# kscalelabs/gym-kmanip

Measured on AMD Instinct MI355X. Metric: env steps/sec (whole node), KManipSoloArm @4096 envs, 1/2/4/8 MI355X, higher is better.
Workload: dtype f64

## Files before the change

### gym_kmanip_amd/csrc/kmanip_api.hip

```cpp
#include <hip/hip_runtime.h>

#include <cstdio>
#include <cstdlib>
#include <cmath>
#include <cstring>
#include <new>
#include <string>
#include <vector>

#include "kmanip_device.hpp"

#define KM_VERSION "kmanip-hip 0.37 (gfx950, f64)"

static thread_local std::string g_create_error;

struct KHandle_ {
  KModelDesc desc;
  KDeviceModel* dmodel = nullptr;
  KDeviceState st{};
  int device = 0;
  int num_envs = 0;
  std::string err;
  std::vector<hipEvent_t> ev;
  std::vector<char> ev_render;
  bool timing = false;
  int timing_every = 1;
  long timing_count = 0;
  double* rd_rec[2] = {nullptr, nullptr};
  int rd_sel = 0;
  int timed_steps = 0;
  double* qpos_snap[2] = {nullptr, nullptr};
  int render_src = -1;
  bool last_step_timed = false;
  int step_cam = -1, step_h = 0, step_w = 0;
  float* step_depth = nullptr;
  int epb_forced = 0;
  int32_t* slot_env = nullptr;
  bool cost_sort = false;
  KCostWeights cost_w{18, 1, 2000, 0, 0, 100};
  uint8_t* spread_flags[2] = {nullptr, nullptr};
  unsigned spread_k = 0;
  int last_epb = 0;
  double* envp_buf = nullptr;
  double* ep_range_buf = nullptr;
  int* ep_flag = nullptr;
  KVisArgs vis{};
  double* vp_buf = nullptr;
  double* vp_range_buf = nullptr;
  int* vp_flag = nullptr;
  int32_t* ep_snap[2] = {nullptr, nullptr};
  bool ep_snap_ok[2] = {false, false};
  std::vector<KLinkCapsule> links;
  KLinkCapsule* links_buf = nullptr;
  bool depth_links = false;
  unsigned long long* index_errors = nullptr;
  double* stage_buf = nullptr;
  int32_t* stage_cnt = nullptr;
  int stage_cap = 0;
  std::vector<void*> allocs;
};

struct DevGuard {
  int prev = -1;
  bool ok = true;
  explicit DevGuard(int dev) {
// ... 1119 lines not shown
```

### gym_kmanip_amd/csrc/kmanip_dyn_newton.hpp

```cpp
#pragma once

enum { KM_SUB_ALL = 0, KM_SUB_ARM = 1, KM_SUB_CUBE = 2 };
template <int NL, int S> struct SubSet {
  static constexpr int D0 = S == KM_SUB_CUBE ? NL : 0, D1 = S == KM_SUB_ARM ? NL : NL + 6;
  static constexpr int kind(int c) { return slot_kind<NL>(c); }
  static constexpr bool slot(int c) { return S == KM_SUB_ALL || (S == KM_SUB_ARM ? kind(c) == 2 : kind(c) == 0); }
  static constexpr int c0(int c) { const int k = kind(c); const int lo = k == 0 ? NL : 0; return lo > D0 ? lo : D0; }
  static constexpr int c1(int c) { const int k = kind(c); const int hi = k == 2 ? NL : NL + 6; return hi < D1 ? hi : D1; }
};

template <int G, int N, int D0, int D1>
__device__ __forceinline__ void chol_rows(real (&h)[N], real& invd, int sub, int& bad) {
  static_for<D0, D1>([&](auto kc) {
    constexpr int k = decltype(kc)::value;
    real dk = gbcast<G, k>(h[k]);
    if (!(dk > 0)) { bad = 1; dk = 1; }
    const real inv = rsqrt_nr(dk);
    const real lik = h[k] * inv;
    h[k] = lik;
    if (sub == k) invd = inv;
    const BSrc<G> lsrc = bsrc<G>(lik);
    fnmac_cols<G, k + 1, D1>(h, lsrc, lik);
    if constexpr (k + 2 >= D1 && k + 1 < D1) dpp_settle(h[k + 1]);
  });
// ... 20 lines not shown
__device__ __forceinline__ void chol_rows1(real (&h)[N], real (&ut)[N], real& invd, int sl, bool live, int& bad) {
  invd = 0;
  if constexpr (UT) {
#pragma unroll
    for (int j = 0; j < N; j++) ut[j] = 0;
  }
  static_for<D0, D1>([&](auto kc) {
    constexpr int k = decltype(kc)::value, kl = k - BASE;
    const real dk = gbcast<16, kl>(h[k]);
    bad |= live && !(dk > 0);
    const real inv = rsqrt_nr(dk);
    const bool me = sl == kl;
    const real lik = sl > kl ? h[k] * inv : 0.0;
    h[k] = lik;
    invd = me ? inv : invd;
    if constexpr (UT) {
      const real isk = me ? 1.0 : 0.0;
      static_for<k + 1, D1>([&](auto jc) {
        constexpr int j = decltype(jc)::value;
        dppfma_pn<j - BASE, j == k + 1>(ut[j], lik, isk, h[j], lik, lik);
      });
    } else {
      static_for<k + 1, D1>([&](auto jc) {
        constexpr int j = decltype(jc)::value;
        dppfma1<true, j - BASE, j == k + 1>(h[j], lik, lik);
      });
    }
    if constexpr (k + 2 >= D1 && k + 1 < D1) dpp_settle(h[k + 1]);
  });
}
template <int N, int D0, int D1, int BASE, class LT>
__device__ __forceinline__ void chol_transpose(LT& lt, const real (&h)[N], real (&ut)[N], int sl) {
  const int r = sl < 0 ? 0 : sl;
#pragma unroll
  for (int k = D0; k < D1; k++) lt[r][k - D0] = h[k];
  GSYNC();
  const int col = r + BASE - D0 < 0 ? 0 : (r + BASE - D0 > D1 - D0 - 1 ? D1 - D0 - 1 : r + BASE - D0);
#pragma unroll
  for (int k = D0; k < D1; k++) ut[k] = lt[k - BASE][col];
  GSYNC();
}
template <int N, int D0, int D1, int BASE>
__device__ __forceinline__ real chol_solve_rows1(const real (&h)[N], const real (&ut)[N], real invd, real b) {
  static_for<D0, D1>([&](auto kc) {
    constexpr int k = decltype(kc)::value;
    const real t = b * invd;
    fnmac_bcast16<k - BASE>(b, t, h[k]);
  });
  real z = b * invd;
  static_for<D0, D1>([&](auto kc) {
    constexpr int k = D1 - 1 - (decltype(kc)::value - D0);
    const real t = z * invd;
    fnmac_bcast16<k - BASE>(z, t, ut[k]);
  });
  return z * invd;
}

__device__ __forceinline__ void row_ls(int type, real x, real y, real R, real Dn, real fl, real& d1, real& d2) {
  if (type == 0) {
    if (x <= -R * fl) d1 += -fl * y;
    else if (x >= R * fl) d1 += fl * y;
    else { d1 += Dn * x * y; d2 += Dn * y * y; }
  } else if (x < 0) { d1 += Dn * x * y; d2 += Dn * y * y; }
}
__device__ __forceinline__ real row_eval(int type, real x, real R, real Dn, real fl, real& f, int& quad) {
  if (type == 0) {
    if (x <= -R * fl) { f = fl; quad = 0; return fl * (-0.5 * R * fl - x); }
    if (x >= R * fl) { f = -fl; quad = 0; return fl * (-0.5 * R * fl + x); }
    f = -Dn * x; quad = 1; return 0.5 * Dn * x * x;
  }
  if (x < 0) { f = -Dn * x; quad = 1; return 0.5 * Dn * x * x; }
  f = 0; quad = 0; return 0;
}

template <int NL, int G>
__device__ __forceinline__ void cube_part(const Ws<NL>& w, real x, real* lin, real* angw) {
  lin[0] = gbcast<G, NL>(x); lin[1] = gbcast<G, NL + 1>(x); lin[2] = gbcast<G, NL + 2>(x);
  const real ab[3] = {gbcast<G, NL + 3>(x), gbcast<G, NL + 4>(x), gbcast<G, NL + 5>(x)};
  mat_vec3(angw, w.k.cube_mat, ab);
}
template <int NL>
__device__ __forceinline__ void plane_proj(const Ws<NL>& w, int c, const real* lin, const real* angw, real* u) {
  const real r[3] = {w.c_pos[c][0] - w.qpos[NL], w.c_pos[c][1] - w.qpos[NL + 1], w.c_pos[c][2] - w.qpos[NL + 2]};
  real v[3];
  cross3(v, angw, r);
  v[0] += lin[0]; v[1] += lin[1]; v[2] += lin[2];
  u[0] = v[2]; u[1] = v[1]; u[2] = -v[0]; u[3] = angw[2];
}

template <int NL>
__device__ __forceinline__ void plane_proj_lane(const Ws<NL>& w, int sub, const real* lin, const real* angw, real* u) {
  plane_proj<NL>(w, sub < 4 ? sub : 0, lin, angw, u);
}

template <int NL, int G>
__device__ __forceinline__ void build_constraints_newton(Ws<NL>& w, const LModel<NL>& lm, const KModelDesc* m, int sub,
                                                         CReg<NL>& cr, real invm) {
  SlotC& sc = cr.sc;
  constexpr int NV = Dim<NL>::NV, NC = Dim<NL>::NC, NSPH = Dim<NL>::NSPH;
  cr.fl = 0; cr.Rf = 1; cr.Df = 1; cr.areff = 0; cr.sg = 0; cr.Rl = 1; cr.Dl = 1; cr.arefl = 0;
  const bool armlane = sub < NL, cubelane = sub >= NL && sub < NV;
  const int jl = armlane ? sub : 0, ce = cubelane ? sub - NL : 0;
  const int si = sub < NL ? sub : NL - 1, sv = sub < NV ? sub : NV - 1, ck = ce >= 3 ? ce - 3 : 0;
  const int cs = sub < NC ? sub : NC - 1;
  real dofw = lm.dofw[si], cubew0 = KM_EP_CUBEW(w, lm, 0), cubew1 = KM_EP_CUBEW(w, lm, 1), qvs = w.qvel[sv], kk0 = lm.kb[0][0], bb0 = lm.kb[0][1];
  real floss = lm.floss[si], imp00 = lm.imp0[0], qps = w.qpos[si], rlo = lm.range[si][0], rhi = lm.range[si][1], distc = w.c_dist[cs];
// ... 266 lines not shown
                                                  const real (&W)[7], real (&h)[Dim<NL>::NV], bool in, uint32_t act, bool joint) {
  constexpr int NV = Dim<NL>::NV, NC = Dim<NL>::NC, J0 = CUBECOLS ? NL : 0;
  using SS = SubSet<NL, S>;
  {
    real dg = sub < NL ? 0.0 : mdiag;
    if (qf) dg += cr.Df;
    if (ql) dg += cr.Dl;
    const real idg = joint ? 1.0 : 0.0;
#pragma unroll
    for (int j = J0; j < NV; j++) h[j] = in ? (j < NL ? cr.mrow[j] : 0.0) + ((j == sub) ? dg : 0.0) : ((j == sub) ? idg : 0.0);
  }
  real Wb[7];
#pragma unroll
  for (int i = 0; i < 7; i++) Wb[i] = row0<G>(W[i]);
  static_for<0, NC>([&](auto cc) {
    constexpr int c = decltype(cc)::value;
    if constexpr (SS::slot(c)) {
      if ((act >> c) & 1u) {
        const real j0 = cr.jb[c][0], j1 = cr.jb[c][1], j2 = cr.jb[c][2], j3 = cr.jb[c][3];
        real t0 = 0, t1 = 0, t2 = 0, t3 = 0;
        if constexpr (SS::kind(c) != 2) {
          dppfma_acc4<c>(t0, Wb[0], j0, Wb[1], j1, Wb[2], j2, Wb[3], j3);
          dppfma3<false, c, c, c>(t1, Wb[1], j0, t2, Wb[2], j0, t3, Wb[3], j0);
          dppfma3<false, c, c, c, false>(t1, Wb[4], j1, t2, Wb[5], j2, t3, Wb[6], j3);
        } else {
          dppfma_acc3<c>(t0, Wb[0], j0, Wb[1], j1, Wb[2], j2);
          dppfma2<false, c, c>(t1, Wb[1], j0, t2, Wb[2], j0);
          dppfma2<false, c, c, false>(t1, Wb[4], j1, t2, Wb[5], j2);
        }
        const BSrc<G> j0s = bsrc<G>(j0), j1s = bsrc<G>(j1), j2s = bsrc<G>(j2), j3s = bsrc<G>(j3);
        static_for<(SS::c0(c) > J0 ? SS::c0(c) : J0), SS::c1(c)>([&](auto jc) {
          constexpr int j = decltype(jc)::value;
          constexpr bool WT = G == 32 && j == SS::c0(c);
          if constexpr (SS::kind(c) != 2) dppfma_acc4<j & 15, WT>(h[j], bsel<G, j>(j0s), t0, bsel<G, j>(j1s), t1, bsel<G, j>(j2s), t2, bsel<G, j>(j3s), t3);
          else dppfma_acc3<j & 15, WT>(h[j], bsel<G, j>(j0s), t0, bsel<G, j>(j1s), t1, bsel<G, j>(j2s), t2);
        });
      }
    }
  });
}

template <int NL, int G, int S, bool JOINT = false>
__device__ __forceinline__ void newton_loop_sl(Ws<NL>& w, const LModel<NL>& lm, const KModelDesc* m, int sub, const CReg<NL>& cr,
                                               real mdiag, real a_s, real& a, real& Mr, real cost, real& grad, int& qf, int& ql,
                                               real (&u)[4], real (&W)[7], Prof& pf, bool two = false, real cost_b = 0, int iter0 = 0,
                                               int* resume = nullptr, real* rcost = nullptr, int* riter = nullptr) {
  static_assert(!JOINT || (S == KM_SUB_ALL && G == 16), "the joint loop is the whole-problem loop of the one-row groups");
  constexpr int NV = Dim<NL>::NV, NC = Dim<NL>::NC, NSS = Dim<NL>::NSS;
  using SS = SubSet<NL, S>;
  const SlotC& sc = cr.sc;
  int prob = (JOINT && two) ? (int)KM_SUB_ARM : S;
  uint32_t act = w.cact;
  bool in = sub >= SS::D0 && sub < SS::D1, slin = slot_lane_in<NL, S>(sub);
  int sig0 = 0;
  bool cache_ok = false;
  real invd_keep = 0;
  auto enter = [&](int pr) {
    constexpr uint32_t ARM_SLOTS = ((1u << NC) - 1u) & ~((1u << (4 + NSS)) - 1u);
    cache_ok = false;
    if constexpr (JOINT) {
      if (pr == KM_SUB_CUBE) {
#pragma unroll
        for (int k = 0; k < NL; k++) w.LT[sub][k] = 0;
        invd_keep = sub < NL ? 1.0 : 0.0; sig0 = 0; cache_ok = true;
      }
    }
    prob = pr;
    act = pr == KM_SUB_ARM ? (w.cact & ARM_SLOTS) : (w.cact & 0xFu);
    in = pr == KM_SUB_ARM ? sub < NL : (sub >= NL && sub < NV);
    slin = pr == KM_SUB_ARM ? (sub >= 4 + NSS && sub < NC) : sub < 4;
  };
  if (JOINT && two) enter(KM_SUB_ARM);
  const real scale = KM_EP_SCALE(w, lm);
  const real tol = m->solver_tolerance;
  const int maxit = m->solver_iterations;
  pf.ph(40);
  auto small = [&]() { const real g0 = in ? grad : 0.0; return km_sqrt(gsum<G>(g0 * g0)) * scale < tol; };
  if (small()) {
    if (!(JOINT && prob == KM_SUB_ARM)) return;
    enter(KM_SUB_CUBE); cost = cost_b;
    if (small()) return;
  }
  for (int iter = iter0; ; iter++) {
    if constexpr (JOINT) {
      if (!__any(!two)) { *resume = prob; *rcost = cost; *riter = iter; return; }
    }
#ifdef KM_PROFILE
    const bool lone_it = JOINT && __popcll(__ballot(1)) <= 16;
    if constexpr (JOINT) pf.it_begin();
#endif
    real p = 0;
    bool plain = false;
    uint32_t rows = 0;
    if (S == KM_SUB_ARM || (JOINT && prob == KM_SUB_ARM)) {
      const unsigned long long bq = __ballot(slin && W[0] != 0);
      const unsigned long long bal = __ballot(in && (qf | ql));
      const int sh = (threadIdx.x & 63) - sub;
      constexpr uint32_t GM = G == 32 ? 0xFFFFFFFFu : 0xFFFFu;
      const bool cq = ((uint32_t)(bq >> sh) & GM) != 0;
      rows = (uint32_t)(bal >> sh) & GM;
      if constexpr (G == 32) {
        const uint32_t lowm = lm.split ? (1u << lm.split) - 1u : 0xFFFFFFFFu;
        plain = !cq && __popc(rows & lowm) <= 2 && __popc(rows & ~lowm) <= 2;
        rows &= (sub < lm.split || !lm.split) ? lowm : ~lowm;
      } else plain = !cq && __popc(rows) <= 2;
    }
    if constexpr (KM_WORK_COUNTERS(NL)) {
      if (sub == 0) w.work += plain ? KM_WORK_PLAIN : (prob == KM_SUB_ALL ? KM_WORK_ALL : (prob == KM_SUB_ARM ? KM_WORK_ARM : KM_WORK_CUBE));
    }
    if (plain) {
      const BSrc<G> gs = bsrc<G>(in ? grad : 0.0);
      const int row = sub < NL ? sub : 0;
      real mi[NL];
#pragma unroll
      for (int j = 0; j < NL; j++) mi[j] = w.Minv[row][j];
      const int i1 = rows ? __ffs(rows) - 1 : 0, i2 = (rows & (rows - 1)) ? __ffs(rows & (rows - 1)) - 1 : i1;
      const real m11 = w.Minv[i1][i1], m22 = w.Minv[i2][i2], a12 = w.Minv[i1][i2], r1 = w.Minv[row][i1], r2 = w.Minv[row][i2];
      const real dl = (qf ? cr.Df : 0.0) + (ql ? cr.Dl : 0.0);
      const real d1 = __shfl(dl, i1, G), d2 = __shfl(dl, i2, G);
      real y = 0;
      fmac_rowvec<G, 0, NL>(y, gs, [&](int j) { return mi[j]; });
      real corr = 0;
      if (rows) {
        const real y1 = __shfl(y, i1, G), y2 = __shfl(y, i2, G);
        const real a11 = frcp(d1) + m11;
        real z1, z2 = 0;
        if (i2 == i1) z1 = y1 * frcp(a11);
        else {
          const real a22 = frcp(d2) + m22;
          const real idet = frcp(a11 * a22 - a12 * a12);
          z1 = (a22 * y1 - a12 * y2) * idet;
          z2 = (a11 * y2 - a12 * y1) * idet;
        }
        corr = r1 * z1 + (i2 == i1 ? 0.0 : r2 * z2);
      }
      p = in ? -(y - corr) : 0.0;
      pf.ph(11 + 6 * S);
    } else {
      real h[NV];
      bool partial = false;
      int sig = 0;
      if constexpr (S == KM_SUB_ALL && G == 16) {
        sig = (in && sub < NL ? (qf | ql << 1) : 0)
              | ((slin && sub >= 4 && ((act >> sub) & 1u)) ? (slot_edge_mask(sc, u) & (sc.D3 != 0 ? 0x3F : 0xF)) << 2 : 0);
        const bool same = cache_ok && gor<G>((int)(sig != sig0)) == 0;
        partial = __all(same);
      }
      if constexpr (S == KM_SUB_ALL && G == 16) { if (prob == KM_SUB_ALL) pf.cnt(partial ? 41 : 42, 1); else pf.cnt(43, partial ? 1 : 0x10000); }
      if (partial) newton_hessian_sl<NL, G, S, true>(w, sub, cr, mdiag, qf, ql, W, h, in, act, JOINT);
      else newton_hessian_sl<NL, G, S>(w, sub, cr, mdiag, qf, ql, W, h, in, act, JOINT);
      pf.ph(9 + 6 * S);
      int hbad = 0;
      bool blocks = false;
      if constexpr (S == KM_SUB_ARM && G == 32) blocks = lm.split != 0;
      if (blocks) {
        if constexpr (S == KM_SUB_ARM && G == 32) {
          constexpr int NB = KM_BLOCK_MAX;
          const int split = lm.split, lane0 = (threadIdx.x & 63) & ~31;
          const int row = (threadIdx.x >> 4) & 1, c = threadIdx.x & 15;
          const int base = row ? split : 0, nb = row ? NL - split : split;
          const bool on = c < nb;
          const int src = lane0 + (on ? base + c : 0);
          real mine[NB], loc[NB];
#pragma unroll
          for (int k = 0; k < NB; k++) {
            const real lo = h[k], hi = split == 10 ? h[(10 + k) < NL ? 10 + k : NL - 1] : h[(11 + k) < NL ? 11 + k : NL - 1];
            mine[k] = sub < split ? lo : hi;
          }
          real sv[NB];
#pragma unroll
          for (int k = 0; k < NB; k++) sv[k] = __shfl(mine[k], src, 64);
          real gsrc = __shfl(in ? -grad : 0.0, src, 64);
          static_assert(NB == 11, "the pins below name eleven block columns");
          km_pin(sv[0], sv[1], sv[2], sv[3], sv[4], sv[5]); km_pin(sv[6], sv[7], sv[8], sv[9], sv[10], gsrc);
#pragma unroll
          for (int k = 0; k < NB; k++) loc[k] = (on && k < nb) ? sv[k] : ((!on && k == c) ? 1.0 : 0.0);
          real invl = 0, utl[NB];
          chol_rows1<NB, 0, NB, 0, true>(loc, utl, invl, c, true, hbad);
          if (__any(hbad)) { const int gb = gor<G>(hbad); if (gb && sub == 0) w.bad = 1; }
          pf.ph(10 + 6 * S);
          const real pl = chol_solve_rows1<NB, 0, NB, 0>(loc, utl, invl, on ? gsrc : 0.0);
          const int back = lane0 + (sub < split ? sub : 16 + (sub < NL ? sub - split : 0));
          const real pb = __shfl(pl, back, 64);
          p = in ? pb : 0.0;
        }
      } else {
        constexpr bool onerow = G == 16 || (S == KM_SUB_CUBE && NL >= 16);
        real invd = 0;
        if constexpr (onerow) {
          constexpr int BASE = G == 16 ? 0 : 16, ND = SS::D1 - SS::D0;
          const int sl = sub - BASE;
          const bool live = G == 16 || sub >= 16;
          real ut[NV];
          if constexpr (ND <= 6) {
            chol_rows1<NV, SS::D0, SS::D1, BASE, true>(h, ut, invd, sl, live, hbad);
          } else if constexpr (S == KM_SUB_ALL && G == 16) {
            if (partial) {
#pragma unroll
              for (int k = 0; k < NL; k++) h[k] = w.LT[sub][k];
              static_for<0, NL>([&](auto kc) {
                constexpr int k = decltype(kc)::value;
                fnmac_cols<16, NL, NV, NV, true>(h, bsrc<16>(h[k]), h[k]);
              });
              dpp_settle(h[NL]);
              real invc = 0;
              chol_rows1<NV, NL, NV, 0, false>(h, ut, invc, sl, live, hbad);
              invd = sub < NL ? invd_keep : invc;
#pragma unroll
              for (int k = NL; k < NV; k++) w.LT[sub][k] = h[k];
              GSYNC();
#pragma unroll
              for (int k = 0; k < NV; k++) ut[k] = w.LT[k][sub];
              GSYNC();
            } else {
              chol_rows1<NV, SS::D0, SS::D1, BASE, false>(h, ut, invd, sl, live, hbad);
              chol_transpose<NV, SS::D0, SS::D1, BASE>(w.LT, h, ut, sl);
              invd_keep = invd; sig0 = sig; cache_ok = true;
            }
          } else {
            chol_rows1<NV, SS::D0, SS::D1, BASE, false>(h, ut, invd, sl, live, hbad);
            chol_transpose<NV, SS::D0, SS::D1, BASE>(w.LT, h, ut, sl);
          }
          if (hbad && sub == 0) w.bad = 1;
          pf.ph(10 + 6 * S);
          p = chol_solve_rows1<NV, SS::D0, SS::D1, BASE>(h, ut, invd, in ? -grad : 0.0);
        } else {
          chol_rows<G, NV, SS::D0, SS::D1>(h, invd, sub, hbad);
          if (hbad && sub == 0) w.bad = 1;
          pf.ph(10 + 6 * S);
          p = chol_solve_rows<G, NV, SS::D0, SS::D1>(h, invd, sub, in ? -grad : 0.0);
        }
      }
      pf.ph(11 + 6 * S);
    }
    real Mp;
    if constexpr (S == KM_SUB_CUBE) Mp = mdiag * p; else Mp = mass_mul<NL, G>(cr, sub, mdiag, p);
    real s3[3] = {in ? p * Mr : 0.0, p * Mp, in ? p * grad : 0.0};
    gsum_n<G, 3>(s3);
    const real gp = s3[0], pMp = s3[1], d10 = s3[2];
    real y[4];
    slot_project<NL, G, S>(w, cr, act, sub, p, y);
    if (!slin) { y[0] = 0; y[1] = 0; y[2] = 0; y[3] = 0; }
    const real xf = a - cr.areff, xl = cr.sg * a - cr.arefl, yl = cr.sg * p;
    pf.ph(12 + 6 * S);
    real alpha = 0, lo = 0, hi = INFINITY;
    if (d10 < 0) {
      alpha = 1;
      for (int it = 0; it < 50; it++) {
        real e1 = 0, e2 = 0;
        if (in && cr.fl > 0) row_ls(0, xf + alpha * p, p, cr.Rf, cr.Df, cr.fl, e1, e2);
        if (in && cr.sg != 0) row_ls(1, xl + alpha * yl, yl, cr.Rl, cr.Dl, 0.0, e1, e2);
        const real X[4] = {u[0] + alpha * y[0], u[1] + alpha * y[1], u[2] + alpha * y[2], u[3] + alpha * y[3]};
        slot_ls(sc, X, y, e1, e2);
        real e12[2] = {e1, e2};
        gsum_n<G, 2>(e12);
        const real d1 = gp + alpha * pMp + e12[0];
        const real d2 = pMp + e12[1];
        if (fabs(d1) <= 1e-8 * fabs(d10)) break;
        if (d1 < 0) lo = alpha; else hi = alpha;
        if (hi - lo <= 1e-14 * hi) break;
        if (it == 49) break;
        real an = alpha - d1 * frcp(d2);
        if (!(an > lo && an < hi)) an = isfinite(hi) ? 0.5 * (lo + hi) : 2 * alpha + 1;
        alpha = an;
      }
    }
    pf.ph(13 + 6 * S);
    a += alpha * p;
    Mr += alpha * Mp;
#pragma unroll
    for (int k = 0; k < 4; k++) u[k] += alpha * y[k];
    real F[4];
    const real cslot = slot_eval<true>(sc, u, F, W);
    real cl = slin ? cslot : 0.0;
    if (in) {
      cl += 0.5 * (a - a_s) * Mr;
      grad = Mr;
      qf = 0; ql = 0;
      if (cr.fl > 0) { real f; cl += row_eval(0, a - cr.areff, cr.Rf, cr.Df, cr.fl, f, qf); grad -= f; }
      if (cr.sg != 0) { real f; cl += row_eval(1, cr.sg * a - cr.arefl, cr.Rl, cr.Dl, 0.0, f, ql); grad -= cr.sg * f; }
    }
    real gsl = grad;
    slot_grad<NL, G, S>(cr, act, F, gsl);
    if (in) grad = gsl;
    const real g1 = in ? grad : 0.0;
    real cg[2] = {cl, g1 * g1};
    gsum_n<G, 2>(cg);
    const real cost_new = cg[0];
    const real improvement = scale * (cost - cost_new), gradient = scale * km_sqrt(cg[1]);
    cost = cost_new;
    pf.ph(14 + 6 * S);
#ifdef KM_PROFILE
    if constexpr (JOINT) { if (prob == KM_SUB_ALL) { pf.cnt(lone_it ? 44 : 45, 1); pf.it_end(lone_it ? 46 : 47); } }
#endif
    if (improvement < tol || gradient < tol || w.bad || iter + 1 >= maxit) {
      if (!(JOINT && prob == KM_SUB_ARM)) break;
      enter(KM_SUB_CUBE); cost = cost_b;
      if (small()) break;
      iter = -1;
    }
  }
}

template <int NL, int G>
__device__ __forceinline__ real solve_newton_sl(Ws<NL>& w, const LModel<NL>& lm, const KModelDesc* m, int sub, CReg<NL>& cr, real a_s,
                                                real invm, Prof& pf) {
  constexpr int NV = Dim<NL>::NV;
  const uint32_t act = w.cact;
  const real warm = sub < NV ? w.warm[sub] : 0.0;
  const real mdiag = (sub >= NL && sub < NV) ? 1.0 / invm : 0.0;
  real grad; int qf, ql;
  real u[4], W[7];
  real c0, c1, csl;
  real a = warm;
  real Mr = mass_mul<NL, G>(cr, sub, mdiag, warm - a_s);
  newton_eval_sl<NL, G, true>(w, sub, cr, a, a_s, Mr, grad, qf, ql, u, W, c0, c1, csl);
  real c3[3] = {csl, c0, c1};
  gsum_n<G, 3>(c3);
  const real cs = c3[0];
  real cost0 = c3[1], cost1 = c3[2];
  pf.ph(8);
  if (!(cost0 + cost1 < cs)) {
    a = a_s; Mr = 0;
    real dummy;
    newton_eval_sl<NL, G, false>(w, sub, cr, a, a_s, Mr, grad, qf, ql, u, W, c0, c1, dummy);
    real c2[2] = {c0, c1};
    gsum_n<G, 2>(c2);
    cost0 = c2[0]; cost1 = c2[1];
    pf.ph(38);
  }
  constexpr uint32_t FC_MASK = ((1u << Dim<NL>::NSS) - 1u) << 4;
  const bool coupled = (act & FC_MASK) != 0;
// ... 61 lines not shown
```

### gym_kmanip_amd/lib.py

```python
from __future__ import annotations

import ctypes as C
import os
import subprocess

from .model import KModelDesc

_HERE = os.path.dirname(os.path.abspath(__file__))
LIB_PATH = os.environ.get("KMANIP_LIB") or os.path.join(_HERE, "libkmanip_hip.so")
_lib = None

EXPORTS = [
    "kmanip_model_desc_size", "kmanip_create", "kmanip_reset", "kmanip_step", "kmanip_step_chunk", "kmanip_get_state",
    "kmanip_set_state", "kmanip_get_episode", "kmanip_set_episode", "kmanip_get_counters", "kmanip_bind_sim_time", "kmanip_bind_applied_force", "kmanip_bind_reward_done_record", "kmanip_select_reward_done_record", "kmanip_observe", "kmanip_forces", "kmanip_kinematics", "kmanip_set_seed", "kmanip_get_diag", "kmanip_timing_summary", "kmanip_enable_timing", "kmanip_ik", "kmanip_ik_eval",
    "kmanip_render_depth", "kmanip_render_rgb", "kmanip_render_rgb_multi", "kmanip_render_labels_multi", "kmanip_render_seg", "kmanip_set_render_links", "kmanip_get_render_links", "kmanip_set_depth_links", "kmanip_get_depth_links", "kmanip_get_camera_poses", "kmanip_render_points", "kmanip_snapshot_render_state", "kmanip_set_render_source", "kmanip_bind_step_depth", "kmanip_scripted_action", "kmanip_sample_action", "kmanip_set_env_params", "kmanip_get_env_params", "kmanip_set_env_param_ranges", "kmanip_set_visual_params", "kmanip_get_visual_params", "kmanip_set_visual_param_ranges",
    "kmanip_get_state_dev", "kmanip_set_state_dev", "kmanip_copy_envs", "kmanip_state_index_errors", "kmanip_num_envs", "kmanip_last_error", "kmanip_version", "kmanip_destroy",
]


DEBUG_EXPORTS = ["kmanip_dbg_wave_clocks"]


class KManipError(RuntimeError):
    pass


class KLinkCapsule(C.Structure):
    _fields_ = [("link", C.c_int32), ("label", C.c_int32), ("cam_mask", C.c_uint32), ("pad_", C.c_int32),
                ("p0", C.c_double * 3), ("seg", C.c_double * 3), ("radius", C.c_double)]


class KStateDev(C.Structure):
    _fields_ = [("qpos", C.c_void_p), ("qvel", C.c_void_p), ("ctrl", C.c_void_p), ("qacc_warm", C.c_void_p),
                ("step_idx", C.c_void_p), ("episode", C.c_void_p)]


class KForcesDev(C.Structure):
    _fields_ = [("qacc", C.c_void_p), ("qfrc_constraint", C.c_void_p), ("qfrc_actuator", C.c_void_p), ("contact_force", C.c_void_p),
                ("contact_bit", C.c_void_p), ("contact_frame", C.c_void_p), ("contact_pos", C.c_void_p), ("contact_dist", C.c_void_p),
                ("contact_mask", C.c_void_p), ("status", C.c_void_p)]


class KKinDev(C.Structure):
    _fields_ = [("link_xpos", C.c_void_p), ("link_xmat", C.c_void_p), ("site_xpos", C.c_void_p), ("site_xmat", C.c_void_p),
                ("site_jacp", C.c_void_p), ("site_jacr", C.c_void_p), ("site_vel", C.c_void_p), ("qM", C.c_void_p),
                ("qfrc_bias", C.c_void_p), ("status", C.c_void_p)]


KM_MAX_LINK_CAPSULES = 24
KM_COPY_EPISODE, KM_COPY_ENV_PARAMS = 1, 2
KM_POINTS_FRAMES = {"camera": 0, "world": 1}


def build(force: bool = False) -> str:
    src_dir = os.path.join(_HERE, "csrc")
    cmd = ["make", "-C", src_dir, "-s", "-j4"] + (["-B"] if force else [])
    subprocess.check_call(cmd)
    return LIB_PATH


def load():
    global _lib
    if _lib is not None:
        return _lib
    if not os.path.exists(LIB_PATH):
        raise KManipError(
            "libkmanip_hip.so is not built (%s). Run `python -c 'import __graft_entry__ as g; g.build()'`; "
            "there is no CPU fallback for the simulation path." % LIB_PATH)
    try:
        import torch
    except Exception:
        pass
    lib = C.CDLL(LIB_PATH)
    vp, i32p, u8p, f64p, f32p = C.c_void_p, C.POINTER(C.c_int32), C.POINTER(C.c_uint8), C.POINTER(C.c_double), C.POINTER(C.c_float)
    lib.kmanip_model_desc_size.restype = C.c_int
    lib.kmanip_create.argtypes = [C.POINTER(KModelDesc), C.c_int, C.c_int, C.c_uint64, C.c_int64, C.POINTER(vp)]
    lib.kmanip_reset.argtypes = [vp, vp, vp, vp]
    lib.kmanip_step.argtypes = [vp, vp, vp, vp, vp, vp]
    lib.kmanip_step_chunk.argtypes = [vp, C.c_int, vp, vp, vp, vp, vp]
    lib.kmanip_get_state.argtypes = [vp, f64p, f64p, f64p, f64p, i32p]
    lib.kmanip_set_state.argtypes = [vp, f64p, f64p, f64p, f64p, i32p]
    lib.kmanip_get_episode.argtypes = [vp, i32p]
    lib.kmanip_set_episode.argtypes = [vp, i32p]
    lib.kmanip_get_counters.argtypes = [vp, vp, vp, vp]
    lib.kmanip_bind_sim_time.argtypes = [vp, vp]
    lib.kmanip_bind_applied_force.argtypes = [vp, vp]
    lib.kmanip_bind_reward_done_record.argtypes = [vp, vp, vp]
    lib.kmanip_select_reward_done_record.argtypes = [vp, C.c_int]
    lib.kmanip_observe.argtypes = [vp, vp, vp, vp]
    lib.kmanip_forces.argtypes = [vp, C.POINTER(KForcesDev), vp]
    lib.kmanip_kinematics.argtypes = [vp, C.POINTER(KKinDev), vp]
    lib.kmanip_set_seed.argtypes = [vp, C.c_uint64, C.c_int]
    lib.kmanip_get_diag.argtypes = [vp, C.POINTER(C.c_uint32), i32p, i32p]
    lib.kmanip_timing_summary.argtypes = [vp, f64p, f64p, f64p, i32p]
    lib.kmanip_enable_timing.argtypes = [vp, C.c_int]
    lib.kmanip_ik.argtypes = [vp, C.c_int, C.c_int, f64p, f64p, f64p, f64p, i32p, i32p]
    lib.kmanip_ik_eval.argtypes = [vp, C.c_int, C.c_int, f64p, f64p, f64p, f64p, f64p]
    lib.kmanip_render_depth.argtypes = [vp, C.c_int, C.c_int, C.c_int, vp, vp]
    lib.kmanip_render_rgb.argtypes = [vp, C.c_int, C.c_int, C.c_int, vp, vp]
    lib.kmanip_render_rgb_multi.argtypes = [vp, C.c_int, i32p, i32p, i32p, C.POINTER(vp), vp]
    lib.kmanip_render_labels_multi.argtypes = [vp, C.c_int, i32p, i32p, i32p, C.POINTER(vp), C.POINTER(vp), vp]
    lib.kmanip_render_seg.argtypes = [vp, C.c_int, C.c_int, C.c_int, vp, vp]
    lib.kmanip_set_render_links.argtypes = [vp, C.c_int, C.POINTER(KLinkCapsule)]
    lib.kmanip_get_render_links.argtypes = [vp, C.POINTER(C.c_int), C.POINTER(KLinkCapsule)]
    lib.kmanip_set_depth_links.argtypes = [vp, C.c_int]
    lib.kmanip_get_depth_links.argtypes = [vp, C.POINTER(C.c_int)]
    lib.kmanip_get_camera_poses.argtypes = [vp, C.c_int, vp, vp]
    lib.kmanip_render_points.argtypes = [vp, C.c_int, C.c_int, C.c_int, C.c_int, vp, vp, vp]
    lib.kmanip_snapshot_render_state.argtypes = [vp, C.c_int, vp]
# ... 27 lines not shown
```

### gym_kmanip_amd/csrc/kmanip_dyn_tree.hpp

```cpp
#pragma once
template <int NL, int G>
__device__ __forceinline__ void fk_parallel(Ws<NL>& w, const LModel<NL>& lm, int sub, real* kin = nullptr) {
  real R[9] = {0, 0, 0, 0, 0, 0, 0, 0, 0}, p[3] = {0, 0, 0};
  const bool on = sub < NL;
  const int li = on ? sub : 0;
  real q = w.qpos[li], lp[3] = {lm.pos[li][0], lm.pos[li][1], lm.pos[li][2]}, lR[9], cl[3] = {lm.com[li][0], lm.com[li][1], lm.com[li][2]};
#pragma unroll
  for (int c = 0; c < 9; c++) lR[c] = lm.R[li][c];
  int jt = lm.jtype[li], jmp0 = lm.jump[0][li], jmp1 = lm.jump[1][li], jmp2 = lm.jump[2][li], jmp3 = lm.jump[3][li], rounds = lm.fk_rounds;
  km_pin(q); km_pin(lp, cl); km_pin(lR); km_pin_i(jt, rounds); km_pin_i(jmp0, jmp1); km_pin_i(jmp2, jmp3);
  if (on) {
    p[0] = lp[0]; p[1] = lp[1]; p[2] = lp[2];
    if (jt == KM_JNT_SLIDE) {
#pragma unroll
      for (int c = 0; c < 9; c++) R[c] = lR[c];
      p[0] += R[2] * q; p[1] += R[5] * q; p[2] += R[8] * q;
    } else {
      real sn, cs;
      km_sincos(q, &sn, &cs);
#pragma unroll
      for (int a = 0; a < 3; a++) {
        const real c0 = lR[3 * a], c1 = lR[3 * a + 1];
        R[3 * a] = cs * c0 + sn * c1;
        R[3 * a + 1] = cs * c1 - sn * c0;
        R[3 * a + 2] = lR[3 * a + 2];
      }
    }
#pragma unroll
    for (int c = 0; c < 9; c++) w.k.xmat[sub][c] = R[c];
    w.k.xpos[sub][0] = p[0]; w.k.xpos[sub][1] = p[1]; w.k.xpos[sub][2] = p[2];
  } else if (sub == NL) {
    real cq[4] = {w.qpos[NL + 3], w.qpos[NL + 4], w.qpos[NL + 5], w.qpos[NL + 6]}, cm[9];
    normalize4_fast(cq);
    quat2mat(cm, cq);
#pragma unroll
    for (int c = 0; c < 9; c++) w.k.cube_mat[c] = cm[c];
  }
  GSYNC();
  for (int k = 0; k < rounds; k++) {
    const int jk = k == 0 ? jmp0 : (k == 1 ? jmp1 : (k == 2 ? jmp2 : jmp3));
    const int a = on ? jk : -1;
    if (a >= 0) {
      real A[9], pa[3], Rn[9], t[3];
#pragma unroll
      for (int c = 0; c < 9; c++) A[c] = w.k.xmat[a][c];
      pa[0] = w.k.xpos[a][0]; pa[1] = w.k.xpos[a][1]; pa[2] = w.k.xpos[a][2];
      mat_vec3(t, A, p);
      p[0] = t[0] + pa[0]; p[1] = t[1] + pa[1]; p[2] = t[2] + pa[2];
#pragma unroll
      for (int i = 0; i < 3; i++)
#pragma unroll
        for (int j = 0; j < 3; j++) Rn[3 * i + j] = A[3 * i] * R[j] + A[3 * i + 1] * R[3 + j] + A[3 * i + 2] * R[6 + j];
#pragma unroll
      for (int c = 0; c < 9; c++) R[c] = Rn[c];
    }
    GSYNC();
    if (a >= 0) {
#pragma unroll
      for (int c = 0; c < 9; c++) w.k.xmat[sub][c] = R[c];
      w.k.xpos[sub][0] = p[0]; w.k.xpos[sub][1] = p[1]; w.k.xpos[sub][2] = p[2];
    }
    GSYNC();
  }
  real cpo[3] = {0, 0, 0};
  if (on) {
    real cw[3];
    mat_vec3(cw, R, cl);
    cpo[0] = p[0] + cw[0]; cpo[1] = p[1] + cw[1]; cpo[2] = p[2] + cw[2];
    w.k.cpos[sub][0] = cpo[0]; w.k.cpos[sub][1] = cpo[1]; w.k.cpos[sub][2] = cpo[2];
    w.k.axis[sub][0] = R[2]; w.k.axis[sub][1] = R[5]; w.k.axis[sub][2] = R[8];
  }
  if (kin) {
#pragma unroll
    for (int c = 0; c < 9; c++) kin[c] = on ? R[c] : 0.0;
#pragma unroll
    for (int c = 0; c < 3; c++) { kin[9 + c] = on ? p[c] : 0.0; kin[12 + c] = cpo[c]; }
  }
  GSYNC();
}

template <int NL>
__device__ __forceinline__ void com_jac_col(const Ws<NL>& w, const LModel<NL>& lm, int b, int j, real* jv, real* jw) {
  if (lm.jtype[j] == KM_JNT_SLIDE) {
    jv[0] = w.k.axis[j][0]; jv[1] = w.k.axis[j][1]; jv[2] = w.k.axis[j][2];
    jw[0] = 0; jw[1] = 0; jw[2] = 0;
  } else {
    real r[3] = {w.k.cpos[b][0] - w.k.xpos[j][0], w.k.cpos[b][1] - w.k.xpos[j][1], w.k.cpos[b][2] - w.k.xpos[j][2]};
    real ax[3] = {w.k.axis[j][0], w.k.axis[j][1], w.k.axis[j][2]};
    cross3(jv, ax, r);
    jw[0] = ax[0]; jw[1] = ax[1]; jw[2] = ax[2];
  }
}

template <int NL, int G>
__device__ __forceinline__ void composite_own(Ws<NL>& w, const LModel<NL>& lm, int sub) {
  for (int b = sub; b < NL; b += G) {
    const real mb = lm.mass[b];
    const real c[3] = {w.k.cpos[b][0], w.k.cpos[b][1], w.k.cpos[b][2]};
    const real* R = w.k.xmat[b];
    const real I0 = lm.inertia[b][0], I1 = lm.inertia[b][1], I2 = lm.inertia[b][2];
    const real cc = dot3(c, c);
    real* o = w.f.comp[b];
    o[0] = mb; o[1] = mb * c[0]; o[2] = mb * c[1]; o[3] = mb * c[2];
    o[4] = R[0] * R[0] * I0 + R[1] * R[1] * I1 + R[2] * R[2] * I2 + mb * (cc - c[0] * c[0]);
    o[5] = R[0] * R[3] * I0 + R[1] * R[4] * I1 + R[2] * R[5] * I2 - mb * c[0] * c[1];
    o[6] = R[0] * R[6] * I0 + R[1] * R[7] * I1 + R[2] * R[8] * I2 - mb * c[0] * c[2];
    o[7] = R[3] * R[3] * I0 + R[4] * R[4] * I1 + R[5] * R[5] * I2 + mb * (cc - c[1] * c[1]);
    o[8] = R[3] * R[6] * I0 + R[4] * R[7] * I1 + R[5] * R[8] * I2 - mb * c[1] * c[2];
    o[9] = R[6] * R[6] * I0 + R[7] * R[7] * I1 + R[8] * R[8] * I2 + mb * (cc - c[2] * c[2]);
  }
}
template <int NL, int G>
__device__ __forceinline__ void composite_accumulate(Ws<NL>& w, const LModel<NL>& lm, int sub) {
  real acc[16];
  const bool on = sub < NL;
  if (on) {
    if constexpr (NL <= 10) {
    const uint32_t dm = lm.desc[sub];
#pragma unroll
    for (int k = 0; k < 16; k++) acc[k] = 0;
// ... 88 lines not shown
    const real mb = on ? massb : 0.0;
    const real* R = Rk;
    const real cc = dot3(c, c);
    own[0] = mb; own[1] = mb * c[0]; own[2] = mb * c[1]; own[3] = mb * c[2];
    own[4] = R[0] * R[0] * I0 + R[1] * R[1] * I1 + R[2] * R[2] * I2 + mb * (cc - c[0] * c[0]);
    own[5] = R[0] * R[3] * I0 + R[1] * R[4] * I1 + R[2] * R[5] * I2 - mb * c[0] * c[1];
    own[6] = R[0] * R[6] * I0 + R[1] * R[7] * I1 + R[2] * R[8] * I2 - mb * c[0] * c[2];
    own[7] = R[3] * R[3] * I0 + R[4] * R[4] * I1 + R[5] * R[5] * I2 + mb * (cc - c[1] * c[1]);
    own[8] = R[3] * R[6] * I0 + R[4] * R[7] * I1 + R[5] * R[8] * I2 - mb * c[1] * c[2];
    own[9] = R[6] * R[6] * I0 + R[7] * R[7] * I1 + R[8] * R[8] * I2 + mb * (cc - c[2] * c[2]);
#pragma unroll
    for (int k = 0; k < 6; k++) own[10 + k] = FN[k];
    if (!on) {
#pragma unroll
      for (int k = 0; k < 16; k++) own[k] = 0;
    }
  }
  real acc[16];
#pragma unroll
  for (int k = 0; k < 16; k++) acc[k] = 0;
  const uint32_t dm = on ? descb >> base : 0u;
  static_for<0, W>([&](auto jc) {
    constexpr int j = decltype(jc)::value;
    const real take = ((dm >> j) & 1u) ? 1.0 : 0.0;
    constexpr bool WT = j == 0;
    dppfma4<false, j, j, j, j, WT>(acc[0], own[0], take, acc[1], own[1], take, acc[2], own[2], take, acc[3], own[3], take);
    dppfma4<false, j, j, j, j, WT>(acc[4], own[4], take, acc[5], own[5], take, acc[6], own[6], take, acc[7], own[7], take);
    dppfma4<false, j, j, j, j, WT>(acc[8], own[8], take, acc[9], own[9], take, acc[10], own[10], take, acc[11], own[11], take);
    dppfma4<false, j, j, j, j, WT>(acc[12], own[12], take, acc[13], own[13], take, acc[14], own[14], take, acc[15], own[15], take);
  });
  if (on) {
    const int j = li;
    const real* o = acc;
    const real ax[3] = {Rk[2], Rk[5], Rk[8]};
    const real h[3] = {o[1], o[2], o[3]};
    real F[3], N[3], t[3];
    const bool slide = jtb == KM_JNT_SLIDE;
    if (slide) {
      F[0] = o[0] * ax[0]; F[1] = o[0] * ax[1]; F[2] = o[0] * ax[2];
      cross3(N, h, ax);
    } else {
      real aO[3];
      cross3(aO, oj, ax);
      cross3(t, ax, h);
      F[0] = o[0] * aO[0] + t[0]; F[1] = o[0] * aO[1] + t[1]; F[2] = o[0] * aO[2] + t[2];
      N[0] = o[4] * ax[0] + o[5] * ax[1] + o[6] * ax[2];
      N[1] = o[5] * ax[0] + o[7] * ax[1] + o[8] * ax[2];
      N[2] = o[6] * ax[0] + o[8] * ax[1] + o[9] * ax[2];
      cross3(t, h, aO);
      N[0] += t[0]; N[1] += t[1]; N[2] += t[2];
    }
    const uint32_t am = ancb;
    real mcol[W];
#pragma unroll
    for (int c = 0; c < W; c++) {
      const int i = base + c < NL ? base + c : NL - 1;
      const real ai[3] = {w.k.axis[i][0], w.k.axis[i][1], w.k.axis[i][2]};
      const real oi[3] = {w.k.xpos[i][0], w.k.xpos[i][1], w.k.xpos[i][2]};
      cross3(t, oi, F);
      const real mo[3] = {N[0] - t[0], N[1] - t[1], N[2] - t[2]};
      const real val = lm.jtype[i] == KM_JNT_SLIDE ? dot3(ai, F) : dot3(ai, mo);
      mcol[c] = ((am >> i) & 1u) ? val : 0.0;
    }
    __builtin_amdgcn_sched_group_barrier(0x100, 8 * W, 0);
    __builtin_amdgcn_sched_group_barrier(0x002, 64 * W, 0);
#pragma unroll
    for (int c = 0; c < W; c++) {
      const int i = base + c;
      if (W != NL && i >= NL) continue;
      real* const up = i <= j ? &w.Minv[i][j] : &w.tmp[j];
      real* const lo = i <= j ? &w.Minv[j][i] : &w.tmp[j];
      *up = mcol[c];
      *lo = mcol[c];
    }
    const real Fb[3] = {acc[10], acc[11], acc[12]};
    if (slide) w.bias[j] = dot3(ax, Fb);
    else {
      cross3(t, oj, Fb);
      const real mo[3] = {acc[13] - t[0], acc[14] - t[1], acc[15] - t[2]};
      w.bias[j] = dot3(ax, mo);
    }
  }
}

template <int NL, int G>
__device__ __forceinline__ void mass_symmetrize(Ws<NL>& w, int sub) {
  for (int j = sub; j < NL; j += G)
    for (int i = j + 1; i < NL; i++) w.Minv[i][j] = w.Minv[j][i];
}

template <int NL, int G>
__device__ __forceinline__ void bias_bodies_parallel(Ws<NL>& w, const LModel<NL>& lm, const KModelDesc* m, int sub) {
  real* wvb = &w.f.bsc[0][0];
  real* czb = wvb + 3 * NL;
  real* dbb = czb + 3 * NL;
  const bool on = sub < NL;
  const bool slide = on && lm.jtype[sub] == KM_JNT_SLIDE;
  const uint32_t up = on ? (lm.anc[sub] & ~(1u << sub)) : 0u;
  real ax[3] = {0, 0, 0};
  if (on) {
    const real qv = w.qvel[sub];
    ax[0] = w.k.axis[sub][0] * qv; ax[1] = w.k.axis[sub][1] * qv; ax[2] = w.k.axis[sub][2] * qv;
    wvb[3 * sub] = slide ? 0.0 : ax[0]; wvb[3 * sub + 1] = slide ? 0.0 : ax[1]; wvb[3 * sub + 2] = slide ? 0.0 : ax[2];
  }
  GSYNC();
  real wp[3] = {0, 0, 0}, cz[3] = {0, 0, 0};
  if (on) {
#pragma unroll KM_TREE_UNROLL(NL)
    for (int j = 0; j < NL; j++) {
      const bool take = (up >> j) & 1u;
      const real v0 = wvb[3 * j], v1 = wvb[3 * j + 1], v2 = wvb[3 * j + 2];
      wp[0] += take ? v0 : 0.0; wp[1] += take ? v1 : 0.0; wp[2] += take ? v2 : 0.0;
    }
    cross3(cz, wp, ax);
    czb[3 * sub] = slide ? 0.0 : cz[0]; czb[3 * sub + 1] = slide ? 0.0 : cz[1]; czb[3 * sub + 2] = slide ? 0.0 : cz[2];
  }
  GSYNC();
  real alp[3] = {0, 0, 0};
// ... 279 lines not shown
```

Baseline: 7.802 million.

## Cache Cholesky factor in scratch for 32-lane groups, refactor only contact block

```diff
diff --git a/gym_kmanip_amd/csrc/kmanip_api.hip b/gym_kmanip_amd/csrc/kmanip_api.hip
--- a/gym_kmanip_amd/csrc/kmanip_api.hip
+++ b/gym_kmanip_amd/csrc/kmanip_api.hip
@@ -10,7 +10,7 @@
 
 #include "kmanip_device.hpp"
 
-#define KM_VERSION "kmanip-hip 0.37 (gfx950, f64)"
+#define KM_VERSION "kmanip-hip 0.38 (gfx950, f64)"
 
 static thread_local std::string g_create_error;
 
diff --git a/gym_kmanip_amd/csrc/kmanip_dyn_newton.hpp b/gym_kmanip_amd/csrc/kmanip_dyn_newton.hpp
--- a/gym_kmanip_amd/csrc/kmanip_dyn_newton.hpp
+++ b/gym_kmanip_amd/csrc/kmanip_dyn_newton.hpp
@@ -96,6 +96,51 @@
     constexpr int k = D1 - 1 - (decltype(kc)::value - D0);
     const real t = z * invd;
     fnmac_bcast16<k - BASE>(z, t, ut[k]);
+  });
+  return z * invd;
+}
+
+template <int G, int N, int D0, int D1>
+__device__ __forceinline__ void chol_rows_m(real (&h)[N], real& invd, int sub, int& bad) {
+  static_for<D0, D1>([&](auto kc) {
+    constexpr int k = decltype(kc)::value;
+    real dk = gbcast<G, k>(h[k]);
+    if (!(dk > 0)) { bad = 1; dk = 1; }
+    const real inv = rsqrt_nr(dk);
+    const real lik = sub > k ? h[k] * inv : 0.0;
+    h[k] = lik;
+    invd = sub == k ? inv : invd;
+    if constexpr (k + 1 < D1) {
+      const BSrc<G> lsrc = bsrc<G>(lik);
+      fnmac_cols<G, k + 1, D1>(h, lsrc, lik);
+    }
+    if constexpr (k + 2 >= D1 && k + 1 < D1) dpp_settle(h[k + 1]);
+  });
+}
+template <int NL> struct LT2 {
+  static constexpr int NV = Dim<NL>::NV, H = (NV + 1) / 2, LD = NV | 1;
+  static_assert(sizeof(Ws<NL>::k) >= H * LD * sizeof(real) && sizeof(Ws<NL>::f) >= (NV - H) * LD * sizeof(real), "the factor fits the dead scratch");
+  static __device__ __forceinline__ real* row(Ws<NL>& w, int i) {
+    return i < H ? reinterpret_cast<real*>(&w.k) + i * LD : reinterpret_cast<real*>(&w.f) + (i - H) * LD;
+  }
+};
+template <int N, int D1>
+__device__ __forceinline__ real chol_forward_rows2(const real (&h)[N], real invd, real b) {
+  static_for<0, D1 - 1>([&](auto kc) {
+    constexpr int k = decltype(kc)::value;
+    const real t = b * invd;
+    if constexpr (k < 16) fnmac_bcast16<k>(b, bsrc<32>(t).e, h[k]);
+    else fnmac_bcast16<k - 16>(b, t, h[k]);
+  });
+  return b * invd;
+}
+template <int N, int D1>
+__device__ __forceinline__ real chol_backward_rows2(const real (&ut)[N], real invd, real z) {
+  static_for<0, D1 - 1>([&](auto kc) {
+    constexpr int k = D1 - 1 - decltype(kc)::value;
+    const real t = z * invd;
+    if constexpr (k >= 16) fnmac_bcast16<k - 16>(z, bsrc<32>(t).o, ut[k]);
+    else fnmac_bcast16<k>(z, t, ut[k]);
   });
   return z * invd;
 }
@@ -468,7 +513,7 @@
   int prob = (JOINT && two) ? (int)KM_SUB_ARM : S;
   uint32_t act = w.cact;
   bool in = sub >= SS::D0 && sub < SS::D1, slin = slot_lane_in<NL, S>(sub);
-  int sig0 = 0;
+  int sig0 = G == 32 ? -1 : 0;
   bool cache_ok = false;
   real invd_keep = 0;
   auto enter = [&](int pr) {
@@ -505,6 +550,12 @@
     const bool lone_it = JOINT && __popcll(__ballot(1)) <= 16;
     if constexpr (JOINT) pf.it_begin();
 #endif
+    real flo = 0;
+    if constexpr (G == 32 && S == KM_SUB_ALL) { flo = cr.fl; asm volatile("" : "+v"(flo)); }
+    auto fl_row = [&]() -> real { if constexpr (G == 32 && S == KM_SUB_ALL) return flo; else return cr.fl; };
+    SlotC sco;
+    if constexpr (G == 32 && S == KM_SUB_ALL) { sco = cr.sc; asm volatile("" : "+v"(sco.mu), "+v"(sco.mu3)); }
+    auto sc_eval = [&]() -> const SlotC& { if constexpr (G == 32 && S == KM_SUB_ALL) return sco; else return sc; };
     real p = 0;
     bool plain = false;
     uint32_t rows = 0;
@@ -562,9 +613,23 @@
         const bool same = cache_ok && gor<G>((int)(sig != sig0)) == 0;
         partial = __all(same);
       }
+      if constexpr (S == KM_SUB_ALL && G == 32) {
+        sig = (in && sub < NL ? (qf | ql << 1) : 0)
+              | ((slin && sub >= 4 && ((act >> sub) & 1u)) ? (slot_edge_mask(sc, u) & (sc.D3 != 0 ? 0x3F : 0xF)) << 2 : 0);
+#ifndef KM_NO_PARTIAL32
+        partial = gor<G>((int)(sig != sig0)) == 0;
+#endif
+        pf.cnt(partial ? 41 : 42, 1);
+      }
       if constexpr (S == KM_SUB_ALL && G == 16) { if (prob == KM_SUB_ALL) pf.cnt(partial ? 41 : 42, 1); else pf.cnt(43, partial ? 1 : 0x10000); }
-      if (partial) newton_hessian_sl<NL, G, S, true>(w, sub, cr, mdiag, qf, ql, W, h, in, act, JOINT);
-      else newton_hessian_sl<NL, G, S>(w, sub, cr, mdiag, qf, ql, W, h, in, act, JOINT);
+      if constexpr (G == 32 && S == KM_SUB_ALL) {
+        int subh = sub; asm volatile("" : "+v"(subh));
+        if (partial) newton_hessian_sl<NL, G, S, true>(w, subh, cr, mdiag, qf, ql, W, h, in, act, JOINT);
+        else newton_hessian_sl<NL, G, S>(w, subh, cr, mdiag, qf, ql, W, h, in, act, JOINT);
+      } else {
+        if (partial) newton_hessian_sl<NL, G, S, true>(w, sub, cr, mdiag, qf, ql, W, h, in, act, JOINT);
+        else newton_hessian_sl<NL, G, S>(w, sub, cr, mdiag, qf, ql, W, h, in, act, JOINT);
+      }
       pf.ph(9 + 6 * S);
       int hbad = 0;
       bool blocks = false;
@@ -640,6 +705,41 @@
           if (hbad && sub == 0) w.bad = 1;
           pf.ph(10 + 6 * S);
           p = chol_solve_rows1<NV, SS::D0, SS::D1, BASE>(h, ut, invd, in ? -grad : 0.0);
+        } else if constexpr (S == KM_SUB_ALL) {
+          using LT = LT2<NL>;
+          int sb = sub; asm volatile("" : "+v"(sb));
+          real* const lrow = LT::row(w, sb < NV ? sb : 0);
+          const int col = sb < NV ? sb : NV - 1;
+          if (partial) {
+#pragma unroll
+            for (int k = 0; k < NL; k++) h[k] = lrow[k];
+            static_for<0, NL>([&](auto kc) {
+              constexpr int k = decltype(kc)::value;
+              km_pin(h[k]);
+              fnmac_cols<G, NL, NV, NV, true>(h, bsrc<G>(h[k]), h[k]);
+            });
+            dpp_settle(h[NL]);
+            real invc = 0;
+            chol_rows_m<G, NV, NL, NV>(h, invc, sb, hbad);
+            invd = sb < NL ? lrow[NV] : invc;
+#pragma unroll
+            for (int k = NL; k < NV; k++) lrow[k] = h[k];
+          } else {
+            chol_rows_m<G, NV, 0, NV>(h, invd, sb, hbad);
+#pragma unroll
+            for (int k = 0; k < NV; k++) lrow[k] = h[k];
+            if (sb < NV) lrow[NV] = invd;
+            sig0 = sig;
+          }
+          if (hbad && sub == 0) w.bad = 1;
+          pf.ph(10 + 6 * S);
+          const real z = chol_forward_rows2<NV, NV>(h, invd, in ? -grad : 0.0);
+          GSYNC();
+          real ut[NV];
+#pragma unroll
+          for (int k = 0; k < NV; k++) ut[k] = LT::row(w, k)[col];
+          GSYNC();
+          p = chol_backward_rows2<NV, NV>(ut, invd, z);
         } else {
           chol_rows<G, NV, SS::D0, SS::D1>(h, invd, sub, hbad);
           if (hbad && sub == 0) w.bad = 1;
@@ -664,7 +764,7 @@
       alpha = 1;
       for (int it = 0; it < 50; it++) {
         real e1 = 0, e2 = 0;
-        if (in && cr.fl > 0) row_ls(0, xf + alpha * p, p, cr.Rf, cr.Df, cr.fl, e1, e2);
+        if (in && fl_row() > 0) row_ls(0, xf + alpha * p, p, cr.Rf, cr.Df, fl_row(), e1, e2);
         if (in && cr.sg != 0) row_ls(1, xl + alpha * yl, yl, cr.Rl, cr.Dl, 0.0, e1, e2);
         const real X[4] = {u[0] + alpha * y[0], u[1] + alpha * y[1], u[2] + alpha * y[2], u[3] + alpha * y[3]};
         slot_ls(sc, X, y, e1, e2);
@@ -687,13 +787,13 @@
 #pragma unroll
     for (int k = 0; k < 4; k++) u[k] += alpha * y[k];
     real F[4];
-    const real cslot = slot_eval<true>(sc, u, F, W);
+    const real cslot = slot_eval<true>(sc_eval(), u, F, W);
     real cl = slin ? cslot : 0.0;
     if (in) {
       cl += 0.5 * (a - a_s) * Mr;
       grad = Mr;
       qf = 0; ql = 0;
-      if (cr.fl > 0) { real f; cl += row_eval(0, a - cr.areff, cr.Rf, cr.Df, cr.fl, f, qf); grad -= f; }
+      if (fl_row() > 0) { real f; cl += row_eval(0, a - cr.areff, cr.Rf, cr.Df, fl_row(), f, qf); grad -= f; }
       if (cr.sg != 0) { real f; cl += row_eval(1, cr.sg * a - cr.arefl, cr.Rl, cr.Dl, 0.0, f, ql); grad -= cr.sg * f; }
     }
     real gsl = grad;
diff --git a/gym_kmanip_amd/lib.py b/gym_kmanip_amd/lib.py
--- a/gym_kmanip_amd/lib.py
+++ b/gym_kmanip_amd/lib.py
@@ -54,7 +54,7 @@
 
 def build(force: bool = False) -> str:
     src_dir = os.path.join(_HERE, "csrc")
-    cmd = ["make", "-C", src_dir, "-s", "-j4"] + (["-B"] if force else [])
+    cmd = ["make", "-C", src_dir, "-s", "-j4", "all", "nopartial"] + (["-B"] if force else [])
     subprocess.check_call(cmd)
     return LIB_PATH
 
```

New measurement: 7.776 million. No clear change (-0.3%).

## Use cross-lane permutes for FK chain and mass-matrix column broadcasts

Applied to the files above, without the earlier changes.

```diff
diff --git a/gym_kmanip_amd/csrc/kmanip_api.hip b/gym_kmanip_amd/csrc/kmanip_api.hip
--- a/gym_kmanip_amd/csrc/kmanip_api.hip
+++ b/gym_kmanip_amd/csrc/kmanip_api.hip
@@ -10,7 +10,7 @@
 
 #include "kmanip_device.hpp"
 
-#define KM_VERSION "kmanip-hip 0.37 (gfx950, f64)"
+#define KM_VERSION "kmanip-hip 0.38 (gfx950, f64)"
 
 static thread_local std::string g_create_error;
 
diff --git a/gym_kmanip_amd/csrc/kmanip_dyn_tree.hpp b/gym_kmanip_amd/csrc/kmanip_dyn_tree.hpp
--- a/gym_kmanip_amd/csrc/kmanip_dyn_tree.hpp
+++ b/gym_kmanip_amd/csrc/kmanip_dyn_tree.hpp
@@ -1,6 +1,35 @@
 #pragma once
+__device__ __forceinline__ real lane_gather(int addr, real v) {
+  const int lo = __builtin_amdgcn_ds_bpermute(addr, __double2loint(v)), hi = __builtin_amdgcn_ds_bpermute(addr, __double2hiint(v));
+  return __hiloint2double(hi, lo);
+}
+__device__ __forceinline__ real dot3_pinned(real a0, real b0, real a1, real b1, real a2, real b2) {
+#pragma clang fp contract(off)
+  const real m = a1 * b1;
+  return __builtin_fma(a2, b2, __builtin_fma(a0, b0, m));
+}
+__device__ __forceinline__ real dot3_pinned(const real* a, const real* b) { return dot3_pinned(a[0], b[0], a[1], b[1], a[2], b[2]); }
+__device__ __forceinline__ real diff2_pinned(real a, real b, real c, real d) {
+#pragma clang fp contract(off)
+  const real m = c * d;
+  return __builtin_fma(a, b, -m);
+}
+__device__ __forceinline__ real sum2_pinned(real a, real b, real c, real d) {
+#pragma clang fp contract(off)
+  const real m = c * d;
+  return __builtin_fma(a, b, m);
+}
+__device__ __forceinline__ void cross3_pinned(real* r, const real* a, const real* b) {
+  const real x = diff2_pinned(a[1], b[2], a[2], b[1]), y = diff2_pinned(a[2], b[0], a[0], b[2]), z = diff2_pinned(a[0], b[1], a[1], b[0]);
+  r[0] = x; r[1] = y; r[2] = z;
+}
+__device__ __forceinline__ void mat_vec3_pinned(real* r, const real* m, const real* v) {
+  const real x = dot3_pinned(m[0], v[0], m[1], v[1], m[2], v[2]), y = dot3_pinned(m[3], v[0], m[4], v[1], m[5], v[2]), z = dot3_pinned(m[6], v[0], m[7], v[1], m[8], v[2]);
+  r[0] = x; r[1] = y; r[2] = z;
+}
 template <int NL, int G>
 __device__ __forceinline__ void fk_parallel(Ws<NL>& w, const LModel<NL>& lm, int sub, real* kin = nullptr) {
+  constexpr bool ROW = G == 16 && NL <= 10;
   real R[9] = {0, 0, 0, 0, 0, 0, 0, 0, 0}, p[3] = {0, 0, 0};
   const bool on = sub < NL;
   const int li = on ? sub : 0;
@@ -21,14 +50,21 @@
 #pragma unroll
       for (int a = 0; a < 3; a++) {
         const real c0 = lR[3 * a], c1 = lR[3 * a + 1];
-        R[3 * a] = cs * c0 + sn * c1;
-        R[3 * a + 1] = cs * c1 - sn * c0;
+        if constexpr (ROW) {
+          R[3 * a] = sum2_pinned(cs, c0, sn, c1);
+          R[3 * a + 1] = diff2_pinned(cs, c1, sn, c0);
+        } else {
+          R[3 * a] = cs * c0 + sn * c1;
+          R[3 * a + 1] = cs * c1 - sn * c0;
+        }
         R[3 * a + 2] = lR[3 * a + 2];
       }
     }
-#pragma unroll
-    for (int c = 0; c < 9; c++) w.k.xmat[sub][c] = R[c];
-    w.k.xpos[sub][0] = p[0]; w.k.xpos[sub][1] = p[1]; w.k.xpos[sub][2] = p[2];
+    if constexpr (!ROW) {
+#pragma unroll
+      for (int c = 0; c < 9; c++) w.k.xmat[sub][c] = R[c];
+      w.k.xpos[sub][0] = p[0]; w.k.xpos[sub][1] = p[1]; w.k.xpos[sub][2] = p[2];
+    }
   } else if (sub == NL) {
     real cq[4] = {w.qpos[NL + 3], w.qpos[NL + 4], w.qpos[NL + 5], w.qpos[NL + 6]}, cm[9];
     normalize4_fast(cq);
@@ -36,6 +72,32 @@
 #pragma unroll
     for (int c = 0; c < 9; c++) w.k.cube_mat[c] = cm[c];
   }
+  if constexpr (ROW) {
+    const int nrounds = __builtin_amdgcn_readfirstlane(rounds);
+    const int row4 = (threadIdx.x & 48) << 2;
+    for (int k = 0; k < nrounds; k++) {
+      const int jk = k == 0 ? jmp0 : (k == 1 ? jmp1 : (k == 2 ? jmp2 : jmp3));
+      const int a = on ? jk : -1;
+      const int src = row4 + (((a >= 0 ? a : 0) & 15) << 2);
+      real A[9], pa[3];
+#pragma unroll
+      for (int c = 0; c < 9; c++) A[c] = lane_gather(src, R[c]);
+#pragma unroll
+      for (int c = 0; c < 3; c++) pa[c] = lane_gather(src, p[c]);
+      km_pin(pa, A);
+      if (a >= 0) {
+        real Rn[9], t[3];
+        mat_vec3_pinned(t, A, p);
+        p[0] = t[0] + pa[0]; p[1] = t[1] + pa[1]; p[2] = t[2] + pa[2];
+#pragma unroll
+        for (int i = 0; i < 3; i++)
+#pragma unroll
+          for (int j = 0; j < 3; j++) Rn[3 * i + j] = dot3_pinned(A[3 * i], R[j], A[3 * i + 1], R[3 + j], A[3 * i + 2], R[6 + j]);
+#pragma unroll
+        for (int c = 0; c < 9; c++) R[c] = Rn[c];
+      }
+    }
+  } else {
   GSYNC();
   for (int k = 0; k < rounds; k++) {
     const int jk = k == 0 ? jmp0 : (k == 1 ? jmp1 : (k == 2 ? jmp2 : jmp3));
@@ -62,10 +124,17 @@
     }
     GSYNC();
   }
+  }
   real cpo[3] = {0, 0, 0};
   if (on) {
     real cw[3];
-    mat_vec3(cw, R, cl);
+    if constexpr (ROW) {
+#pragma unroll
+      for (int c = 0; c < 9; c++) w.k.xmat[sub][c] = R[c];
+      w.k.xpos[sub][0] = p[0]; w.k.xpos[sub][1] = p[1]; w.k.xpos[sub][2] = p[2];
+    }
+    if constexpr (ROW) mat_vec3_pinned(cw, R, cl);
+    else mat_vec3(cw, R, cl);
     cpo[0] = p[0] + cw[0]; cpo[1] = p[1] + cw[1]; cpo[2] = p[2] + cw[2];
     w.k.cpos[sub][0] = cpo[0]; w.k.cpos[sub][1] = cpo[1]; w.k.cpos[sub][2] = cpo[2];
     w.k.axis[sub][0] = R[2]; w.k.axis[sub][1] = R[5]; w.k.axis[sub][2] = R[8];
@@ -260,6 +329,18 @@
     }
     const uint32_t am = ancb;
     real mcol[W];
+    if constexpr (W == NL && NL <= 10) {
+      static_for<0, W>([&](auto cc) {
+        constexpr int i = decltype(cc)::value;
+        const real ai[3] = {gbcast<16, i>(ax[0]), gbcast<16, i>(ax[1]), gbcast<16, i>(ax[2])};
+        const real oi[3] = {gbcast<16, i>(oj[0]), gbcast<16, i>(oj[1]), gbcast<16, i>(oj[2])};
+        const int jti = dpp_i32<0x150 + i>(jtb);
+        cross3_pinned(t, oi, F);
+        const real mo[3] = {N[0] - t[0], N[1] - t[1], N[2] - t[2]};
+        const real val = jti == KM_JNT_SLIDE ? dot3_pinned(ai, F) : dot3_pinned(ai, mo);
+        mcol[i] = ((am >> i) & 1u) ? val : 0.0;
+      });
+    } else {
 #pragma unroll
     for (int c = 0; c < W; c++) {
       const int i = base + c < NL ? base + c : NL - 1;
@@ -272,6 +353,7 @@
     }
     __builtin_amdgcn_sched_group_barrier(0x100, 8 * W, 0);
     __builtin_amdgcn_sched_group_barrier(0x002, 64 * W, 0);
+    }
 #pragma unroll
     for (int c = 0; c < W; c++) {
       const int i = base + c;
```

New measurement: 7.789 million before, 7.903 million after (median of 6 runs). +1.5%, better.
